# itailang/geometric_adv

Hardware: AMD Instinct MI355X
Metric: attack-iterations/sec (B=32, N=2048) at 1/2/4/8 GPUs; Chamfer rel-err vs ref (higher is better)
Workload: dtype f32 (encoder products: f16x2); 1 GPU; BASELINE configs[1]: B=32 random clouds x N=2048, output-space attack (chamfer/chamfer, dist_weight 1.0, lr 0.01), one batch per GPU; batch_per_gpu=32, n_points=2048, global_batch=32, parallelism=batches sharded, dp1, no data-path collective, ranks=1, collective_backend=none, collective_world=1

## Files before the change

### geometric_adv_amd/csrc/decoder.hip

```cpp
#include "ae.h"
#include "decoder_tail.h"
#include "chamfer_grid.h"
#include <limits.h>

namespace geoadv {

int encoder_tiles(const DeviceAE &A, int b);

typedef float f32x16 __attribute__((ext_vector_type(16)));
__device__ __forceinline__ int acc_row16(int reg, int h) { return (reg & 3) + 8 * (reg >> 2) + 4 * h; }

template <int THREADS, int PARTS = 1>
__device__ __forceinline__ void latent_decode_block(const DeviceAE &A, int tiles, const float *pmax, const int *parg,
                                                    const int *pcnt, float *z, int *crit, int *zcnt,
                                                    int *dense, float *d1, float *d2, const int b, const int part_id = 0) {
    __shared__ float gm[8][128];
    __shared__ int ga[8][128], gk[8][128];
    __shared__ float zs[128];
    __shared__ float hs[256];
    __shared__ float part[4][256];
    __shared__ int tie;
    const int t = threadIdx.x;
    GA_STAMP(0, 0);
    if (t == 0) tie = 0;
    for (int g = t >> 7; g < 8; g += THREADS / 128) {
        const int c = t & 127;
        const int tb = tiles * g / 8, te = tiles * (g + 1) / 8;
        float m = -1.f;
        int a = INT_MAX, k = 0;
        constexpr int U = 8;
        for (int t0 = tb; t0 < te; t0 += U) {
            float pm[U];
            int pa[U], pk[U];
#pragma unroll
            for (int u = 0; u < U; ++u) {
                const int tl = t0 + u < te ? t0 + u : te - 1;
                const size_t o = ((size_t)b * tiles + tl) * 128 + c;
                pm[u] = pmax[o]; pa[u] = parg[o]; pk[u] = pcnt[o];
            }
#pragma unroll
            for (int u = 0; u < U; ++u) {
                const bool live = t0 + u < te;
                const bool gt = live && pm[u] > m, eq = live && pm[u] == m;
                k = gt ? pk[u] : (eq ? k + pk[u] : k);
                a = gt ? pa[u] : a;
                m = gt ? pm[u] : m;
            }
        }
        gm[g][c] = m; ga[g][c] = a; gk[g][c] = k;
    }
    __syncthreads();
    GA_STAMP(0, 1);
    if (t < 128) {
        float gmv[8];
        int gav[8], gkv[8];
#pragma unroll
        for (int g = 0; g < 8; ++g) { gmv[g] = gm[g][t]; gav[g] = ga[g][t]; gkv[g] = gk[g][t]; }
        float m = gmv[0];
        int a = gav[0], k = gkv[0];
#pragma unroll
        for (int g = 1; g < 8; ++g) {
            const bool gt = gmv[g] > m, eq = gmv[g] == m;
            k = gt ? gkv[g] : (eq ? k + gkv[g] : k);
            a = gt ? gav[g] : a;
            m = gt ? gmv[g] : m;
        }
        zs[t] = m;
        if (part_id == 0) {
            z[(size_t)b * 128 + t] = m;
            crit[(size_t)b * 128 + t] = a;
            zcnt[(size_t)b * 128 + t] = k;
        }
        if (m > 0.f && k > 1) atomicOr(&tie, 1);
    }
    __syncthreads();
    if (t == 0 && part_id == 0) dense[b] = tie;
    GA_STAMP(0, 2);
    if (!d1) return;
    {
        const float s = fc256_split4<128, THREADS>(zs, A.v0, part);
        if (t < 256) {
            const float v = fmaxf(s + A.c0[t], 0.f);
            hs[t] = v;
            if (part_id == 0) d1[(size_t)b * 256 + t] = v;
        }
    }
    __syncthreads();
    GA_STAMP(0, 3);
    if (PARTS == 1) {
        const float s = fc256_split4<256, THREADS>(hs, A.v1, part);
        if (t < 256) d2[(size_t)b * 256 + t] = fmaxf(s + A.c1[t], 0.f);
    } else {
        constexpr int NC = 256 / PARTS;
        const int col0 = part_id * NC;
        const float s = fc256_split4_cols<256, NC>(hs, A.v1, part, col0);
        if (t < NC) d2[(size_t)b * 256 + col0 + t] = fmaxf(s + A.c1[col0 + t], 0.f);
    }
    GA_STAMP(0, 7);
}

__global__ __launch_bounds__(LD_THREADS) void latent_fc_kernel(DeviceAE A, const float *z, float *d2) {
    __shared__ float zs[128];
    __shared__ float hs[256];
    __shared__ float part[4][256];
    const int t = threadIdx.x, b = blockIdx.x;
    if (t < 128) zs[t] = z[(size_t)b * 128 + t];
    __syncthreads();
    {
        const float s = fc256_split4<128, LD_THREADS>(zs, A.v0, part);
        if (t < 256) hs[t] = fmaxf(s + A.c0[t], 0.f);
    }
    __syncthreads();
    {
        const float s = fc256_split4<256, LD_THREADS>(hs, A.v1, part);
        if (t < 256) d2[(size_t)b * 256 + t] = fmaxf(s + A.c1[t], 0.f);
    }
}

template <int PARTS>
__global__ __launch_bounds__(LD_THREADS) void latent_decode_kernel(DeviceAE A, int tiles, const float *pmax, const int *parg,
                                                                   const int *pcnt, float *z, int *crit, int *zcnt,
                                                                   int *dense, float *d1, float *d2) {
    latent_decode_block<LD_THREADS, PARTS>(A, tiles, pmax, parg, pcnt, z, crit, zcnt, dense, d1, d2, blockIdx.x / PARTS, blockIdx.x % PARTS);
}

template <int THREADS>
__global__ __launch_bounds__(THREADS) void latent_decode_and_grid_kernel(DeviceAE A, int tiles, const float *pmax, const int *parg,
                                                                         const int *pcnt, float *z, int *crit, int *zcnt, int *dense,
                                                                         float *d1, float *d2, int batch, GridArgs G) {
    if ((int)blockIdx.x < batch) {
        latent_decode_block<THREADS>(A, tiles, pmax, parg, pcnt, z, crit, zcnt, dense, d1, d2, blockIdx.x);
        return;
    }
    if (THREADS > GR_THREADS && threadIdx.x >= GR_THREADS) return;
    const int g = blockIdx.x - batch;
    GA_STAMP(1, 0);
    grid_nn_block<GR_MAX_N>(G, g / (2 * GR_QSPLIT), (g / GR_QSPLIT) % 2, g % GR_QSPLIT);
    GA_STAMP(1, 7);
}

__device__ __forceinline__ void decoder_fc2_block(const DeviceAE &A, int batch, const float *d2, float *out, const int cb, const int rb) {
    __shared__ float part[3][16][64];
    GA_STAMP(2, 0);
    const int wave = threadIdx.x >> 6, lane = threadIdx.x & 63;
    const int h = lane >> 5, i = lane & 31;
    const PackedLayer &L = A.dec2_fwd;
    const int kg = L.K >> 3;
    const int per = kg / 4;
    int arow = rb * 32 + i;
    arow = arow < batch ? arow : batch - 1;
    const float *ap = d2 + (size_t)arow * 256 + 4 * h;
    const float4 *bp = reinterpret_cast<const float4 *>(L.w) + (size_t)cb * kg * 64 + lane;
    f32x16 acc = {};
    float4 av[8], wv[8];
#pragma unroll
    for (int u = 0; u < 8; ++u) {
        const int t = wave * per + (u < per ? u : per - 1);
        av[u] = *reinterpret_cast<const float4 *>(ap + 8 * t);
        wv[u] = bp[(size_t)t * 64];
    }
#pragma unroll
    for (int u = 0; u < 8; ++u) {
        if (u < per) {
            acc = __builtin_amdgcn_mfma_f32_32x32x2f32(av[u].x, wv[u].x, acc, 0, 0, 0);
            acc = __builtin_amdgcn_mfma_f32_32x32x2f32(av[u].y, wv[u].y, acc, 0, 0, 0);
            acc = __builtin_amdgcn_mfma_f32_32x32x2f32(av[u].z, wv[u].z, acc, 0, 0, 0);
            acc = __builtin_amdgcn_mfma_f32_32x32x2f32(av[u].w, wv[u].w, acc, 0, 0, 0);
        }
    }
    if (wave > 0) {
#pragma unroll
        for (int r = 0; r < 16; ++r) part[wave - 1][r][lane] = acc[r];
    }
    __syncthreads();
    if (wave == 0) {
        const int ncols = A.dec_dims[GEOADV_DEC_LAYERS];
        const int col = cb * 32 + i;
        const float bias = col < ncols ? A.c2[col] : 0.f;
#pragma unroll
        for (int r = 0; r < 16; ++r) {
            const float v = ((acc[r] + part[0][r][lane]) + part[1][r][lane]) + part[2][r][lane] + bias;
            const int row = rb * 32 + acc_row16(r, h);
            if (row < batch && col < ncols) out[(size_t)row * ncols + col] = v;
        }
    }
    GA_STAMP(2, 7);
}

__global__ __launch_bounds__(256) void decoder_fc2_kernel(DeviceAE A, int batch, const float *d2, float *out, unsigned long long *fill,
                                                         size_t fill_count) {
    if (fill) {
        const size_t stride = (size_t)gridDim.x * gridDim.y * 256;
        for (size_t e = ((size_t)blockIdx.y * gridDim.x + blockIdx.x) * 256 + threadIdx.x; e < fill_count; e += stride) fill[e] = ~0ull;
    }
    decoder_fc2_block(A, batch, d2, out, blockIdx.x, blockIdx.y);
}

constexpr int DB_KC = 64;

__global__ __launch_bounds__(512) void decoder_fc2_bwd_kernel(DeviceAE A, int batch, const float *g_out, float *partial) {
    __shared__ __attribute__((aligned(16))) float as[32 * (DB_KC + 4)];
    GA_STAMP(3, 0);
    const int ch = blockIdx.x, rb = blockIdx.y;
    const int ncols = A.dec_dims[GEOADV_DEC_LAYERS];
    const PackedLayer &L = A.dec2_bwd;
    const int kg_total = L.K >> 3;
    const int k0 = ch * DB_KC;
    const int wave = threadIdx.x >> 6, lane = threadIdx.x & 63;
    const int h = lane >> 5, i = lane & 31;
    const int cb = wave;
    const int t0 = k0 >> 3;
    const int nt = min(DB_KC >> 3, kg_total - t0);
    const float4 *bp = reinterpret_cast<const float4 *>(L.w) + ((size_t)cb * kg_total + t0) * 64 + lane;
    constexpr int NT = DB_KC >> 3;
    float4 wv[NT];
#pragma unroll
    for (int t = 0; t < NT; ++t) wv[t] = bp[(size_t)(t < nt ? t : nt - 1) * 64];
    for (int e = threadIdx.x; e < 32 * DB_KC; e += 512) {
        const int r = e / DB_KC, k = e % DB_KC;
        const int row = rb * 32 + r, kk = k0 + k;
        as[r * (DB_KC + 4) + k] = (row < batch && kk < ncols) ? g_out[(size_t)row * ncols + kk] : 0.f;
    }
    __syncthreads();
    const float *ap = as + i * (DB_KC + 4) + 4 * h;
    f32x16 acc = {};
#pragma unroll
    for (int t = 0; t < NT; ++t) {
        if (t < nt) {
            const float4 a = *reinterpret_cast<const float4 *>(ap + 8 * t);
            acc = __builtin_amdgcn_mfma_f32_32x32x2f32(a.x, wv[t].x, acc, 0, 0, 0);
            acc = __builtin_amdgcn_mfma_f32_32x32x2f32(a.y, wv[t].y, acc, 0, 0, 0);
            acc = __builtin_amdgcn_mfma_f32_32x32x2f32(a.z, wv[t].z, acc, 0, 0, 0);
            acc = __builtin_amdgcn_mfma_f32_32x32x2f32(a.w, wv[t].w, acc, 0, 0, 0);
        }
    }
    const int col = cb * 32 + i;
#pragma unroll
    for (int r = 0; r < 16; ++r) {
        const int row = rb * 32 + acc_row16(r, h);
        if (row < batch) partial[((size_t)ch * batch + row) * 256 + col] = acc[r];
    }
    GA_STAMP(3, 7);
}

__global__ __launch_bounds__(LD_THREADS) void decoder_bwd_tail_kernel(DeviceAE A, int batch, int chunks, const float *partial,
                                                                     const float *d1, const float *d2, float *dz, JacApply ja) {
    decoder_bwd_tail_body(A, batch, chunks, partial, d1, d2, dz, ja, blockIdx.x, nullptr, 0u);
}

int launch_latent_decode(const DeviceAE &A, int b, const float *pmax, const int *parg, const int *pcnt, float *z,
                         int *crit, int *zcnt, int *dense, float *d1, float *d2, hipStream_t stream) {
    if (b <= 0) return GEOADV_OK;
    const int tiles = encoder_tiles(A, b);
    if (d1 && 4 * b <= kCUs) latent_decode_kernel<4><<<4 * b, LD_THREADS, 0, stream>>>(A, tiles, pmax, parg, pcnt, z, crit, zcnt, dense, d1, d2);
    else if (d1 && 2 * b <= kCUs) latent_decode_kernel<2><<<2 * b, LD_THREADS, 0, stream>>>(A, tiles, pmax, parg, pcnt, z, crit, zcnt, dense, d1, d2);
    else latent_decode_kernel<1><<<b, LD_THREADS, 0, stream>>>(A, tiles, pmax, parg, pcnt, z, crit, zcnt, dense, d1, d2);
    GA_LAUNCH_CHECK();
    return GEOADV_OK;
}

int launch_latent_decode_and_grid(const DeviceAE &A, int b, const float *pmax, const int *parg, const int *pcnt, float *z, int *crit,
                                  int *zcnt, int *dense, float *d1, float *d2, const float *P, const float *Q, float *gd1, int *gi1,
                                  float *gd2, int *gi2, int n, int *need, int call, const float *box, hipStream_t stream) {
    if (b <= 0) return GEOADV_OK;
    static DeviceOnce attr;
    if (int rc = attr.run([]() -> int {
            GA_HIP(hipFuncSetAttribute(reinterpret_cast<const void *>(latent_decode_and_grid_kernel<LD_THREADS>),
                                       hipFuncAttributeMaxDynamicSharedMemorySize, (int)chamfer_grid_lds_bytes(GR_MAX_N)));
            GA_HIP(hipFuncSetAttribute(reinterpret_cast<const void *>(latent_decode_and_grid_kernel<GR_THREADS>),
                                       hipFuncAttributeMaxDynamicSharedMemorySize, (int)chamfer_grid_lds_bytes(GR_MAX_N)));
            return GEOADV_OK;
        })) return rc;
    const GridArgs G{P, Q, gd1, gi1, gd2, gi2, n, need, nullptr, call, box};
    const int blocks = b + b * 2 * GR_QSPLIT;
    if (blocks <= kCUs)
        latent_decode_and_grid_kernel<LD_THREADS><<<blocks, LD_THREADS, chamfer_grid_lds_bytes(n), stream>>>(
            A, encoder_tiles(A, b), pmax, parg, pcnt, z, crit, zcnt, dense, d1, d2, b, G);
    else
        latent_decode_and_grid_kernel<GR_THREADS><<<blocks, GR_THREADS, chamfer_grid_lds_bytes(n), stream>>>(
            A, encoder_tiles(A, b), pmax, parg, pcnt, z, crit, zcnt, dense, d1, d2, b, G);
    GA_LAUNCH_CHECK();
    return GEOADV_OK;
}

int launch_latent_fc(const DeviceAE &A, int b, const float *z, float *d2, hipStream_t stream) {
    if (b <= 0) return GEOADV_OK;
    latent_fc_kernel<<<b, LD_THREADS, 0, stream>>>(A, z, d2);
    GA_LAUNCH_CHECK();
    return GEOADV_OK;
}

int launch_decoder_fc2(const DeviceAE &A, int b, const float *d2, float *recon, hipStream_t stream, unsigned long long *fill, size_t fill_count) {
    if (b <= 0) return GEOADV_OK;
    decoder_fc2_kernel<<<dim3(A.dec2_fwd.N / 32, cdiv(b, 32)), 256, 0, stream>>>(A, b, d2, recon, fill, fill_count);
    GA_LAUNCH_CHECK();
    return GEOADV_OK;
}

int decoder_bwd_chunks(const DeviceAE &A) { return cdiv(A.dec2_bwd.K, DB_KC); }

int launch_decoder_fc2_bwd(const DeviceAE &A, int b, const float *g_recon, float *partial, hipStream_t stream) {
    if (b <= 0) return GEOADV_OK;
    decoder_fc2_bwd_kernel<<<dim3(decoder_bwd_chunks(A), cdiv(b, 32)), 512, 0, stream>>>(A, b, g_recon, partial);
    GA_LAUNCH_CHECK();
    return GEOADV_OK;
}

int launch_decoder_bwd(const DeviceAE &A, int b, const float *g_recon, const float *d1, const float *d2, float *partial,
                       float *dz, hipStream_t stream, const int *crit, const float *jac, const int *dense, float *g_enc) {
    if (b <= 0) return GEOADV_OK;
    const int chunks = decoder_bwd_chunks(A);
    decoder_fc2_bwd_kernel<<<dim3(chunks, cdiv(b, 32)), 512, 0, stream>>>(A, b, g_recon, partial);
    GA_LAUNCH_CHECK();
    decoder_bwd_tail_kernel<<<b, LD_THREADS, 0, stream>>>(A, b, chunks, partial, d1, d2, dz, JacApply{crit, jac, dense, g_enc, A.n_points});
    GA_LAUNCH_CHECK();
    return GEOADV_OK;
}

}
GA_STAMPS_GETTER(geoadv_debug_stamps_decoder)
```

### geometric_adv_amd/csrc/decoder_tail.h

```cpp
#pragma once
#include "ae.h"

namespace geoadv {

constexpr int LD_THREADS = 1024;

template <int K, int THREADS = LD_THREADS>
__device__ __forceinline__ float fc256_split4(const float *in_lds, const float *W , float (*part)[256]) {
    const int t = threadIdx.x, o = t & 255;
    constexpr int PER = K / 4;
#pragma unroll
    for (int ks = t >> 8; ks < 4; ks += THREADS / 256) {
        float w[PER];
#pragma unroll
        for (int k = 0; k < PER; ++k) w[k] = W[(size_t)(ks * PER + k) * 256 + o];
        float s = 0.f;
#pragma unroll
        for (int k = 0; k < PER; ++k) s = fmaf(in_lds[ks * PER + k], w[k], s);
        part[ks][o] = s;
    }
    __syncthreads();
    return ((part[0][o] + part[1][o]) + part[2][o]) + part[3][o];
}

template <int K, int NCOLS>
__device__ __forceinline__ float fc256_split4_cols(const float *in_lds, const float *W , float (*part)[256], const int col0) {
    const int t = threadIdx.x, o = col0 + t % NCOLS, ks = t / NCOLS;
    constexpr int PER = K / 4;
    if (ks < 4) {
        float w[PER];
#pragma unroll
        for (int k = 0; k < PER; ++k) w[k] = W[(size_t)(ks * PER + k) * 256 + o];
        float s = 0.f;
#pragma unroll
        for (int k = 0; k < PER; ++k) s = fmaf(in_lds[ks * PER + k], w[k], s);
        part[ks][o] = s;
    }
    __syncthreads();
    return ((part[0][o] + part[1][o]) + part[2][o]) + part[3][o];
}

struct JacApply { const int *crit; const float *jac; const int *dense; float *g_enc; int n; };
__device__ __forceinline__ bool is_dense_all(const JacApply &ja, int b) { return ja.dense && ja.dense[b] != 0; }

__device__ __forceinline__ void decoder_bwd_tail_body(const DeviceAE &A, int batch, int chunks, const float *partial,
                                                      const float *d1, const float *d2, float *dz, const JacApply &ja,
                                                      const int b, unsigned *ready, unsigned epoch) {
    __shared__ float g2[256];
    __shared__ float g1[256];
    __shared__ float part[8][256];
    __shared__ __attribute__((aligned(16))) float dzs[128], jxs[128], jys[128], jzs[128];
    __shared__ __attribute__((aligned(16))) int crs[128];
    const int t = threadIdx.x, o = t & 255, ks = t >> 8;
    GA_STAMP(4, 0);
    float jx = 0.f, jy = 0.f, jz = 0.f;
    int my_crit = -1, is_dense = 0;
    if (ja.jac && t < 128) {
        const float *jp = ja.jac + ((size_t)b * 128 + t) * 3;
        jx = jp[0]; jy = jp[1]; jz = jp[2];
        my_crit = ja.crit[(size_t)b * 128 + t];
        is_dense = ja.dense[b];
    }
    {
        const int cb = chunks * ks / 4, ce = chunks * (ks + 1) / 4;
        float s = 0.f;
#pragma unroll 8
        for (int ch = cb; ch < ce; ++ch) s += partial[((size_t)ch * batch + b) * 256 + o];
        part[ks][o] = s;
    }
    __syncthreads();
    if (t < 256) {
        const float s = ((part[0][t] + part[1][t]) + part[2][t]) + part[3][t];
        g2[t] = d2[(size_t)b * 256 + t] > 0.f ? s : 0.f;
    }
    __syncthreads();
    GA_STAMP(4, 1);
    {
        const float s = fc256_split4<256>(g2, A.v1t, part);
        __syncthreads();
        if (t < 256) g1[t] = d1[(size_t)b * 256 + t] > 0.f ? s : 0.f;
    }
    __syncthreads();
    GA_STAMP(4, 2);
    {
        const int c = t & 127, k8 = t >> 7;
        float w[32];
#pragma unroll
        for (int k = 0; k < 32; ++k) w[k] = A.v0t[(size_t)(k8 * 32 + k) * 128 + c];
        float s = 0.f;
#pragma unroll
        for (int k = 0; k < 32; ++k) s = fmaf(g1[k8 * 32 + k], w[k], s);
        part[k8][c] = s;
        __syncthreads();
        float r = 0.f;
        if (t < 128) {
            r = part[0][t];
#pragma unroll
            for (int q = 1; q < 8; ++q) r += part[q][t];
            dz[(size_t)b * 128 + t] = r;
        }
        if (ready && is_dense_all(ja, b)) {
            asm volatile("s_waitcnt vmcnt(0)" ::: "memory");
            __syncthreads();
            if (t == 0) {
                __builtin_amdgcn_fence(__ATOMIC_RELEASE, "agent");
                asm volatile("s_waitcnt vmcnt(0)" ::: "memory");
                __hip_atomic_store(ready + b, epoch, __ATOMIC_RELAXED, __HIP_MEMORY_SCOPE_AGENT);
            }
        }
        GA_STAMP(4, 3);
        if (ja.jac) {
            if (t < 128) { dzs[t] = r; crs[t] = my_crit; jxs[t] = jx; jys[t] = jy; jzs[t] = jz; }
            __syncthreads();
            {
                const int ch = t & 127, pq = t >> 7, mine = crs[ch];
                float gx = 0.f, gy = 0.f, gz = 0.f;
                const int4 *c4 = reinterpret_cast<const int4 *>(crs) + 4 * pq;
                const float4 *d4 = reinterpret_cast<const float4 *>(dzs) + 4 * pq, *x4 = reinterpret_cast<const float4 *>(jxs) + 4 * pq;
                const float4 *y4 = reinterpret_cast<const float4 *>(jys) + 4 * pq, *z4 = reinterpret_cast<const float4 *>(jzs) + 4 * pq;
                int4 cc[4]; float4 dd[4], xx[4], yy[4], zz[4];
#pragma unroll
                for (int q = 0; q < 4; ++q) { cc[q] = c4[q]; dd[q] = d4[q]; xx[q] = x4[q]; yy[q] = y4[q]; zz[q] = z4[q]; }
#pragma unroll
                for (int q = 0; q < 4; ++q) {
                    const int ci[4] = {cc[q].x, cc[q].y, cc[q].z, cc[q].w};
                    const float di[4] = {dd[q].x, dd[q].y, dd[q].z, dd[q].w}, xi[4] = {xx[q].x, xx[q].y, xx[q].z, xx[q].w};
                    const float yi[4] = {yy[q].x, yy[q].y, yy[q].z, yy[q].w}, zi[4] = {zz[q].x, zz[q].y, zz[q].z, zz[q].w};
#pragma unroll
                    for (int u = 0; u < 4; ++u) {
                        const float d = ci[u] == mine ? di[u] : 0.f;
                        gx = fmaf(d, xi[u], gx); gy = fmaf(d, yi[u], gy); gz = fmaf(d, zi[u], gz);
                    }
                }
                __syncthreads();
                part[pq][ch] = gx; part[pq][128 + ch] = gy;
                __syncthreads();
                float sx = 0.f, sy = 0.f;
                if (t < 128) {
#pragma unroll
                    for (int q = 0; q < 8; ++q) { sx += part[q][t]; sy += part[q][128 + t]; }
                }
                __syncthreads();
                part[pq][ch] = gz;
                __syncthreads();
                if (t < 128 && !is_dense) {
                    float sz = 0.f;
#pragma unroll
                    for (int q = 0; q < 8; ++q) sz += part[q][t];
                    float *g = ja.g_enc + ((size_t)b * ja.n + my_crit) * 3;
                    g[0] = sx; g[1] = sy; g[2] = sz;
                }
            }
        }
    }
    GA_STAMP(4, 7);
}


struct TailDenseArgs {
    int batch, chunks, n;
    const float *partial, *d1, *d2;
    float *dz;
    JacApply ja;
    const float *adv, *z;
    const int *zcnt, *dense_flag;
    float *g_enc;
    unsigned *ready;
    unsigned epoch;
    int *spin_timeout;
};

}
```

Before: 9045 attack-iterations/sec.

## Hoist loads and cut barriers across latent decode, fc2 and tail kernels

Several decoder kernels issue their global loads earlier and drop shared-memory round trips. Bias values, d1/d2 activations and Jacobian inputs are loaded ahead of the compute that needs them. Empty asm constraints force the latent max-reduction loads to be batched. The fc2 cross-wave reduction is spread across all four waves instead of funnelled through wave 0, and the g_out tile load is vectorised to float4. The tail kernel unrolls its partial-sum reduction and drops two __syncthreads by giving the z component its own shared buffer. The trade-offs are more registers and shared memory, and a change in how the dense/tie flag is read.

```diff
diff --git a/geometric_adv_amd/csrc/decoder.hip b/geometric_adv_amd/csrc/decoder.hip
--- a/geometric_adv_amd/csrc/decoder.hip
+++ b/geometric_adv_amd/csrc/decoder.hip
@@ -8,6 +8,7 @@
 int encoder_tiles(const DeviceAE &A, int b);
 
 typedef float f32x16 __attribute__((ext_vector_type(16)));
+typedef float f32x4 __attribute__((ext_vector_type(4)));
 __device__ __forceinline__ int acc_row16(int reg, int h) { return (reg & 3) + 8 * (reg >> 2) + 4 * h; }
 
 template <int THREADS, int PARTS = 1>
@@ -23,6 +24,9 @@
     const int t = threadIdx.x;
     GA_STAMP(0, 0);
     if (t == 0) tie = 0;
+    constexpr int NC1 = 256 / PARTS;
+    const float bias0 = A.c0[t & 255];
+    const float bias1 = A.c1[part_id * NC1 + (PARTS == 1 ? (t & 255) : t % NC1)];
     for (int g = t >> 7; g < 8; g += THREADS / 128) {
         const int c = t & 127;
         const int tb = tiles * g / 8, te = tiles * (g + 1) / 8;
@@ -39,6 +43,8 @@
                 pm[u] = pmax[o]; pa[u] = parg[o]; pk[u] = pcnt[o];
             }
 #pragma unroll
+            for (int u = 0; u < U; ++u) asm volatile("" : "+v"(pm[u]), "+v"(pa[u]), "+v"(pk[u]));
+#pragma unroll
             for (int u = 0; u < U; ++u) {
                 const bool live = t0 + u < te;
                 const bool gt = live && pm[u] > m, eq = live && pm[u] == m;
@@ -80,7 +86,7 @@
     {
         const float s = fc256_split4<128, THREADS>(zs, A.v0, part);
         if (t < 256) {
-            const float v = fmaxf(s + A.c0[t], 0.f);
+            const float v = fmaxf(s + bias0, 0.f);
             hs[t] = v;
             if (part_id == 0) d1[(size_t)b * 256 + t] = v;
         }
@@ -89,12 +95,12 @@
     GA_STAMP(0, 3);
     if (PARTS == 1) {
         const float s = fc256_split4<256, THREADS>(hs, A.v1, part);
-        if (t < 256) d2[(size_t)b * 256 + t] = fmaxf(s + A.c1[t], 0.f);
+        if (t < 256) d2[(size_t)b * 256 + t] = fmaxf(s + bias1, 0.f);
     } else {
-        constexpr int NC = 256 / PARTS;
+        constexpr int NC = NC1;
         const int col0 = part_id * NC;
         const float s = fc256_split4_cols<256, NC>(hs, A.v1, part, col0);
-        if (t < NC) d2[(size_t)b * 256 + col0 + t] = fmaxf(s + A.c1[col0 + t], 0.f);
+        if (t < NC) d2[(size_t)b * 256 + col0 + t] = fmaxf(s + bias1, 0.f);
     }
     GA_STAMP(0, 7);
 }
@@ -104,16 +110,17 @@
     __shared__ float hs[256];
     __shared__ float part[4][256];
     const int t = threadIdx.x, b = blockIdx.x;
+    const float bias0 = A.c0[t & 255], bias1 = A.c1[t & 255];
     if (t < 128) zs[t] = z[(size_t)b * 128 + t];
     __syncthreads();
     {
         const float s = fc256_split4<128, LD_THREADS>(zs, A.v0, part);
-        if (t < 256) hs[t] = fmaxf(s + A.c0[t], 0.f);
+        if (t < 256) hs[t] = fmaxf(s + bias0, 0.f);
     }
     __syncthreads();
     {
         const float s = fc256_split4<256, LD_THREADS>(hs, A.v1, part);
-        if (t < 256) d2[(size_t)b * 256 + t] = fmaxf(s + A.c1[t], 0.f);
+        if (t < 256) d2[(size_t)b * 256 + t] = fmaxf(s + bias1, 0.f);
     }
 }
 
@@ -139,8 +146,9 @@
     GA_STAMP(1, 7);
 }
 
-__device__ __forceinline__ void decoder_fc2_block(const DeviceAE &A, int batch, const float *d2, float *out, const int cb, const int rb) {
-    __shared__ float part[3][16][64];
+__device__ __forceinline__ void decoder_fc2_block(const DeviceAE &A, int batch, const float *d2, float *out, const int cb, const int rb,
+                                                  unsigned long long *fill = nullptr, size_t fill_count = 0) {
+    __shared__ float part[4][16][64];
     GA_STAMP(2, 0);
     const int wave = threadIdx.x >> 6, lane = threadIdx.x & 63;
     const int h = lane >> 5, i = lane & 31;
@@ -159,6 +167,9 @@
         av[u] = *reinterpret_cast<const float4 *>(ap + 8 * t);
         wv[u] = bp[(size_t)t * 64];
     }
+    const int ncols = A.dec_dims[GEOADV_DEC_LAYERS];
+    const int col = cb * 32 + i;
+    const float bias_ld = A.c2[col < ncols ? col : ncols - 1];
 #pragma unroll
     for (int u = 0; u < 8; ++u) {
         if (u < per) {
@@ -168,32 +179,34 @@
             acc = __builtin_amdgcn_mfma_f32_32x32x2f32(av[u].w, wv[u].w, acc, 0, 0, 0);
         }
     }
-    if (wave > 0) {
-#pragma unroll
-        for (int r = 0; r < 16; ++r) part[wave - 1][r][lane] = acc[r];
-    }
-    __syncthreads();
-    if (wave == 0) {
-        const int ncols = A.dec_dims[GEOADV_DEC_LAYERS];
-        const int col = cb * 32 + i;
-        const float bias = col < ncols ? A.c2[col] : 0.f;
-#pragma unroll
-        for (int r = 0; r < 16; ++r) {
-            const float v = ((acc[r] + part[0][r][lane]) + part[1][r][lane]) + part[2][r][lane] + bias;
-            const int row = rb * 32 + acc_row16(r, h);
-            if (row < batch && col < ncols) out[(size_t)row * ncols + col] = v;
-        }
-    }
-    GA_STAMP(2, 7);
-}
-
-__global__ __launch_bounds__(256) void decoder_fc2_kernel(DeviceAE A, int batch, const float *d2, float *out, unsigned long long *fill,
-                                                         size_t fill_count) {
     if (fill) {
         const size_t stride = (size_t)gridDim.x * gridDim.y * 256;
         for (size_t e = ((size_t)blockIdx.y * gridDim.x + blockIdx.x) * 256 + threadIdx.x; e < fill_count; e += stride) fill[e] = ~0ull;
     }
-    decoder_fc2_block(A, batch, d2, out, blockIdx.x, blockIdx.y);
+#pragma unroll
+    for (int r = 0; r < 16; ++r) part[wave][r][lane] = acc[r];
+    __syncthreads();
+    {
+        float p[4][4];
+#pragma unroll
+        for (int j = 0; j < 4; ++j)
+#pragma unroll
+            for (int q = 0; q < 4; ++q) p[j][q] = part[q][4 * wave + j][lane];
+        const float bias = col < ncols ? bias_ld : 0.f;
+        const int row0 = rb * 32 + 8 * wave + 4 * h;
+        float *op = out + (size_t)row0 * ncols + col;
+#pragma unroll
+        for (int j = 0; j < 4; ++j) {
+            const float v = ((p[j][0] + p[j][1]) + p[j][2]) + p[j][3] + bias;
+            if (row0 + j < batch && col < ncols) op[(size_t)j * ncols] = v;
+        }
+    }
+    GA_STAMP(2, 7);
+}
+
+__global__ __launch_bounds__(256) void decoder_fc2_kernel(DeviceAE A, int batch, const float *d2, float *out, unsigned long long *fill,
+                                                         size_t fill_count) {
+    decoder_fc2_block(A, batch, d2, out, blockIdx.x, blockIdx.y, fill, fill_count);
 }
 
 constexpr int DB_KC = 64;
@@ -214,12 +227,32 @@
     const float4 *bp = reinterpret_cast<const float4 *>(L.w) + ((size_t)cb * kg_total + t0) * 64 + lane;
     constexpr int NT = DB_KC >> 3;
     float4 wv[NT];
+    float4 a4;
+    {
+        const int r = threadIdx.x >> 4, k = (threadIdx.x & 15) * 4;
+        const int row = rb * 32 + r, kk = k0 + k;
+        const float *gp = g_out + (size_t)(row < batch ? row : batch - 1) * ncols;
+        if ((ncols & 3) == 0 && (reinterpret_cast<size_t>(g_out) & 15) == 0) {
+            const f32x4 v = *reinterpret_cast<const f32x4 *>(gp + (kk < ncols ? kk : ncols - 4));
+            a4 = make_float4(v.x, v.y, v.z, v.w);
+        } else {
+            a4.x = gp[kk     < ncols ? kk     : ncols - 1];
+            a4.y = gp[kk + 1 < ncols ? kk + 1 : ncols - 1];
+            a4.z = gp[kk + 2 < ncols ? kk + 2 : ncols - 1];
+            a4.w = gp[kk + 3 < ncols ? kk + 3 : ncols - 1];
+        }
+    }
 #pragma unroll
     for (int t = 0; t < NT; ++t) wv[t] = bp[(size_t)(t < nt ? t : nt - 1) * 64];
-    for (int e = threadIdx.x; e < 32 * DB_KC; e += 512) {
-        const int r = e / DB_KC, k = e % DB_KC;
+    {
+        const int r = threadIdx.x >> 4, k = (threadIdx.x & 15) * 4;
         const int row = rb * 32 + r, kk = k0 + k;
-        as[r * (DB_KC + 4) + k] = (row < batch && kk < ncols) ? g_out[(size_t)row * ncols + kk] : 0.f;
+        const bool live = row < batch;
+        a4.x = live && kk     < ncols ? a4.x : 0.f;
+        a4.y = live && kk + 1 < ncols ? a4.y : 0.f;
+        a4.z = live && kk + 2 < ncols ? a4.z : 0.f;
+        a4.w = live && kk + 3 < ncols ? a4.w : 0.f;
+        *reinterpret_cast<float4 *>(as + r * (DB_KC + 4) + k) = a4;
     }
     __syncthreads();
     const float *ap = as + i * (DB_KC + 4) + 4 * h;
diff --git a/geometric_adv_amd/csrc/decoder_tail.h b/geometric_adv_amd/csrc/decoder_tail.h
--- a/geometric_adv_amd/csrc/decoder_tail.h
+++ b/geometric_adv_amd/csrc/decoder_tail.h
@@ -49,41 +49,49 @@
     __shared__ float g2[256];
     __shared__ float g1[256];
     __shared__ float part[8][256];
+    __shared__ float partz[8][128];
     __shared__ __attribute__((aligned(16))) float dzs[128], jxs[128], jys[128], jzs[128];
     __shared__ __attribute__((aligned(16))) int crs[128];
     const int t = threadIdx.x, o = t & 255, ks = t >> 8;
     GA_STAMP(4, 0);
     float jx = 0.f, jy = 0.f, jz = 0.f;
     int my_crit = -1, is_dense = 0;
-    if (ja.jac && t < 128) {
-        const float *jp = ja.jac + ((size_t)b * 128 + t) * 3;
-        jx = jp[0]; jy = jp[1]; jz = jp[2];
-        my_crit = ja.crit[(size_t)b * 128 + t];
-        is_dense = ja.dense[b];
-    }
+    const float d2v = d2[(size_t)b * 256 + o], d1v = d1[(size_t)b * 256 + o];
     {
         const int cb = chunks * ks / 4, ce = chunks * (ks + 1) / 4;
         float s = 0.f;
-#pragma unroll 8
-        for (int ch = cb; ch < ce; ++ch) s += partial[((size_t)ch * batch + b) * 256 + o];
+        constexpr int U = 24;
+        for (int c0 = cb; c0 < ce; c0 += U) {
+            float v[U];
+#pragma unroll
+            for (int u = 0; u < U; ++u) v[u] = partial[((size_t)(c0 + u < ce ? c0 + u : ce - 1) * batch + b) * 256 + o];
+#pragma unroll
+            for (int u = 0; u < U; ++u) s = c0 + u < ce ? s + v[u] : s;
+        }
         part[ks][o] = s;
     }
     __syncthreads();
     if (t < 256) {
         const float s = ((part[0][t] + part[1][t]) + part[2][t]) + part[3][t];
-        g2[t] = d2[(size_t)b * 256 + t] > 0.f ? s : 0.f;
+        g2[t] = d2v > 0.f ? s : 0.f;
     }
     __syncthreads();
     GA_STAMP(4, 1);
     {
         const float s = fc256_split4<256>(g2, A.v1t, part);
         __syncthreads();
-        if (t < 256) g1[t] = d1[(size_t)b * 256 + t] > 0.f ? s : 0.f;
+        if (t < 256) g1[t] = d1v > 0.f ? s : 0.f;
     }
     __syncthreads();
     GA_STAMP(4, 2);
     {
         const int c = t & 127, k8 = t >> 7;
+        if (ja.jac && t < 128) {
+            const float *jp = ja.jac + ((size_t)b * 128 + t) * 3;
+            jx = jp[0]; jy = jp[1]; jz = jp[2];
+            my_crit = ja.crit[(size_t)b * 128 + t];
+        }
+        if (ja.dense) is_dense = ja.dense[b];
         float w[32];
 #pragma unroll
         for (int k = 0; k < 32; ++k) w[k] = A.v0t[(size_t)(k8 * 32 + k) * 128 + c];
@@ -99,7 +107,10 @@
             for (int q = 1; q < 8; ++q) r += part[q][t];
             dz[(size_t)b * 128 + t] = r;
         }
-        if (ready && is_dense_all(ja, b)) {
+        asm volatile("" : "+v"(is_dense));
+        is_dense = __builtin_amdgcn_readfirstlane(is_dense);
+        const bool tied = is_dense != 0;
+        if (ready && tied) {
             asm volatile("s_waitcnt vmcnt(0)" ::: "memory");
             __syncthreads();
             if (t == 0) {
@@ -132,21 +143,12 @@
                         gx = fmaf(d, xi[u], gx); gy = fmaf(d, yi[u], gy); gz = fmaf(d, zi[u], gz);
                     }
                 }
-                __syncthreads();
-                part[pq][ch] = gx; part[pq][128 + ch] = gy;
-                __syncthreads();
-                float sx = 0.f, sy = 0.f;
-                if (t < 128) {
-#pragma unroll
-                    for (int q = 0; q < 8; ++q) { sx += part[q][t]; sy += part[q][128 + t]; }
-                }
-                __syncthreads();
-                part[pq][ch] = gz;
+                part[pq][ch] = gx; part[pq][128 + ch] = gy; partz[pq][ch] = gz;
                 __syncthreads();
                 if (t < 128 && !is_dense) {
-                    float sz = 0.f;
+                    float sx = 0.f, sy = 0.f, sz = 0.f;
 #pragma unroll
-                    for (int q = 0; q < 8; ++q) sz += part[q][t];
+                    for (int q = 0; q < 8; ++q) { sx += part[q][t]; sy += part[q][128 + t]; sz += partz[q][t]; }
                     float *g = ja.g_enc + ((size_t)b * ja.n + my_crit) * 3;
                     g[0] = sx; g[1] = sy; g[2] = sz;
                 }
```

After: 9387 attack-iterations/sec, median of 6. 3.8% higher.
